# ChenJiahao031008/EAO-Fusion

Hardware: AMD Instinct MI355X
Metric: ORB kpts/s (640x480, 1k feat) + local-BA residuals/s (20 KF x 3k pts) (higher is better)
Workload: dtype u8; 1 GPU; ORBextractor FAST+rBRIEF, 640x480, 8-level pyramid, nFeatures 1000, batch=64 synthetic frames per GPU (BASELINE configs[1]); parallelism=frames sharded per GPU, no data-path collective

## Files before the change

eao_fusion_amd/csrc/orb.hip:

```cpp
#include "orb_internal.h"

using namespace eao::orb;

namespace {

__constant__ __align__(16) signed char c_pattern[1024] = {
#include "orb_pattern.inc"
};

constexpr int kResizeRows = 4;
__device__ __forceinline__ unsigned udot2w(unsigned a, unsigned b) {
    typedef unsigned short us2 __attribute__((ext_vector_type(2)));
    return __builtin_amdgcn_udot2(__builtin_bit_cast(us2, a), __builtin_bit_cast(us2, b), 0u, false);
}

struct ResizeLevel { int w, h, pitch, off; };
struct ResizeArgs {
    ResizeLevel D, S;
    double invX, invY;
    int srcIsInput;
    int pyrFrameBytes;
    int G;
    float invG;
    int frameAffinity;
// ... 465 lines not shown
                const int pos = total + __popcll(km & ((1ull << lane) - 1));
                if (pos < cellCap) out[pos] = (unsigned)(x + 3 + c.offX) | ((unsigned)(y + 3 + c.offY) << 12) | ((unsigned)v << 24);
            }
            total += __popcll(km);
        }
        if (total > 0 || pass == 1) {
            if (lane == 0) cellcnt[slot] = min(total, cellCap);
            return;
        }
    }
#undef QDIV
}

__device__ __forceinline__ int reflect101(int p, int len) {
    while (p < 0 || p >= len) p = p < 0 ? -p : 2 * len - 2 - p;
    return p;
}

typedef unsigned short u16x2 __attribute__((ext_vector_type(2)));
__device__ __forceinline__ unsigned udot2(unsigned a, unsigned b, unsigned c) {
    return __builtin_amdgcn_udot2(__builtin_bit_cast(u16x2, a), __builtin_bit_cast(u16x2, b), c, false);
}

struct BlurEdge {
    int off0;
    bool left;
    unsigned selA, selB, selC;
};

__device__ __forceinline__ BlurEdge blur_edge(int x4, int w) {
    BlurEdge e;
    const int wi = x4 >> 2, wmax = (w - 1) >> 2;
    const int wi0 = min(max(wi - 1, 0), wmax - 2);
    e.off0 = 4 * wi0;
    e.left = wi == 0;
    e.selA = e.selB = e.selC = 0;
#pragma unroll
    for (int k = 0; k < 12; k++) {
        int x = min(max(x4 - 4 + k, -3), w + 2);
        x = x < 0 ? -x : x;
        x = min(x, 2 * w - 2 - x);
        const int m = min(max(x - 4 * wi0, 0), 11);
        if (k < 4) e.selA |= (unsigned)min(m, 7) << (8 * k);
        else {
            const unsigned q = (unsigned)min(max(e.left ? m : m - 4, 0), 7) << (8 * (k & 3));
            if (k < 8) e.selB |= q; else e.selC |= q;
        }
    }
    return e;
}

template <int MODE>
__device__ __forceinline__ void blur_load(const uint8_t* __restrict__ base, unsigned rowOff, int x4, int w, const BlurEdge& e, unsigned L[3]) {
    const uint8_t* row = base + rowOff;
    if (MODE == 0) {
        const unsigned* q = reinterpret_cast<const unsigned*>(base + (rowOff + (unsigned)(x4 - 4)));
        L[0] = q[0]; L[1] = q[1]; L[2] = q[2];
    } else if (MODE == 1) {
        const unsigned* q = reinterpret_cast<const unsigned*>(base + (rowOff + (unsigned)e.off0));
        L[0] = q[0]; L[1] = q[1]; L[2] = q[2];
    } else {
        L[0] = L[1] = L[2] = 0;
#pragma unroll
        for (int k = 1; k < 11; k++) L[k >> 2] |= (unsigned)row[reflect101(x4 - 4 + k, w)] << (8 * (k & 3));
    }
}

template <int MODE>
__device__ __forceinline__ void blur_hpass(const unsigned L[3], const BlurEdge& e, unsigned hres[4]) {
    unsigned W0 = L[0], W1 = L[1], W2 = L[2];
    if (MODE == 1) {
        const unsigned a = e.left ? L[0] : L[1], b = e.left ? L[1] : L[2];
        W0 = __builtin_amdgcn_perm(L[1], L[0], e.selA);
        W1 = __builtin_amdgcn_perm(b, a, e.selB);
        W2 = __builtin_amdgcn_perm(b, a, e.selC);
    }
    constexpr unsigned T0 = 18u | 34u << 8 | 49u << 16 | 55u << 24, T1 = 49u | 34u << 8 | 18u << 16;
    hres[0] = __builtin_amdgcn_udot4(__builtin_amdgcn_alignbyte(W1, W0, 1), T0, __builtin_amdgcn_udot4(__builtin_amdgcn_alignbyte(W2, W1, 1), T1, 0, false), false);
    hres[1] = __builtin_amdgcn_udot4(__builtin_amdgcn_alignbyte(W1, W0, 2), T0, __builtin_amdgcn_udot4(__builtin_amdgcn_alignbyte(W2, W1, 2), T1, 0, false), false);
    hres[2] = __builtin_amdgcn_udot4(__builtin_amdgcn_alignbyte(W1, W0, 3), T0, __builtin_amdgcn_udot4(__builtin_amdgcn_alignbyte(W2, W1, 3), T1, 0, false), false);
    hres[3] = __builtin_amdgcn_udot4(W1, T0, __builtin_amdgcn_udot4(W2, T1, 0, false), false);
}

template <int MODE>
__device__ __forceinline__ void blur_strip(const uint8_t* __restrict__ src, int pitch, uint8_t* __restrict__ dst, int dpitch, int x4, int y0, int w, int h) {
    BlurEdge e = {};
    if (MODE == 1) e = blur_edge(x4, w);
    constexpr int NP = (kBlurRows + 6) / 2;
    constexpr int PF = MODE == 2 ? 1 : 3;
    unsigned raw[NP][2][3];
    auto fetch = [&](int m) {
#pragma unroll
        for (int q = 0; q < 2; q++) {
            int t = y0 - 3 + 2 * m + q;
            t = t < 0 ? -t : t;
            t = min(t, 2 * h - 2 - t);
            blur_load<MODE>(src, __umul24(t, pitch), x4, w, e, raw[m][q]);
        }
    };
#pragma unroll
    for (int m = 0; m < PF; m++) fetch(m);
    unsigned P[4][4];
#pragma unroll
    for (int m = 0; m < NP; m++) {
        if (m + PF < NP) fetch(m + PF);
        unsigned hr[2][4];
        blur_hpass<MODE>(raw[m][0], e, hr[0]);
        blur_hpass<MODE>(raw[m][1], e, hr[1]);
#pragma unroll
        for (int i = 0; i < 4; i++) P[m & 3][i] = hr[0][i] | (hr[1][i] << 16);
        if (m >= 3) {
#pragma unroll
            for (int q = 0; q < 2; q++) {
                const unsigned K0 = q ? 18u << 16 : (18u | 34u << 16), K1 = q ? (34u | 49u << 16) : (49u | 55u << 16),
                               K2 = q ? (55u | 49u << 16) : (49u | 34u << 16), K3 = q ? (34u | 18u << 16) : 18u;
                unsigned sv[4];
#pragma unroll
                for (int i = 0; i < 4; i++)
                    sv[i] = udot2(P[(m - 3) & 3][i], K0, udot2(P[(m - 2) & 3][i], K1, udot2(P[(m - 1) & 3][i], K2, udot2(P[m & 3][i], K3, 32768u))));
                const u16x2 lim = {255, 255};
                const u16x2 pa = __builtin_elementwise_min(__builtin_bit_cast(u16x2, __builtin_amdgcn_perm(sv[1], sv[0], 0x07060302u)), lim);
                const u16x2 pb = __builtin_elementwise_min(__builtin_bit_cast(u16x2, __builtin_amdgcn_perm(sv[3], sv[2], 0x07060302u)), lim);
                const unsigned packed = __builtin_amdgcn_perm(__builtin_bit_cast(unsigned, pb), __builtin_bit_cast(unsigned, pa), 0x06040200u);
                const int y = y0 + 2 * (m - 3) + q;
                *reinterpret_cast<unsigned*>(dst + (unsigned)(__umul24(y, dpitch) + x4)) = packed;
            }
        }
    }
}

__global__ __launch_bounds__(256) void k_blur7(const Geom* __restrict__ g, ImgSrc s, uint8_t* __restrict__ blur, int f0, int src0Aligned, int frameAffinity) {
    const int lane = threadIdx.x & 31;
    int f = blockIdx.y, bxi = blockIdx.x;
    if (frameAffinity) {
        const unsigned b = blockIdx.x + gridDim.x * blockIdx.y, xcd = b & 7, slot = b >> 3;
        f = (int)(xcd + 8 * (slot / gridDim.x)); bxi = (int)(slot % gridDim.x);
    }
    f += f0;
    int l = 0;
    while (l + 1 < g->nlevels && bxi >= g->L[l + 1].tileBase) l++;
    const LevelGeom L = g->L[l];
    const int strip = (bxi - L.tileBase) * kBlurStripsPerWg + (int)(threadIdx.x >> 5);
    const int x4 = (strip % L.tilesX) * kBlurSegW + lane * 4;
    const int y0 = (strip / L.tilesX) * kBlurRows;
    if (x4 >= L.w || y0 >= L.h) return;
    int pitch;
    const uint8_t* src = level_ptr(g, s, l, f, &pitch);
    uint8_t* dst = blur + (long long)f * g->pyrFrameBytes + L.off;
    if (l == 0 && !src0Aligned) blur_strip<2>(src, pitch, dst, L.pitch, x4, y0, L.w, L.h);
    else if (__any(x4 < 4 || x4 + 7 > L.w)) blur_strip<1>(src, pitch, dst, L.pitch, x4, y0, L.w, L.h);
    else blur_strip<0>(src, pitch, dst, L.pitch, x4, y0, L.w, L.h);
}

__device__ __forceinline__ int wave_sum_i32(int v) {
    v += __builtin_amdgcn_update_dpp(0, v, 0xB1, 0xF, 0xF, true);
    v += __builtin_amdgcn_update_dpp(0, v, 0x4E, 0xF, 0xF, true);
    v += __builtin_amdgcn_update_dpp(0, v, 0x141, 0xF, 0xF, true);
    v += __builtin_amdgcn_update_dpp(0, v, 0x140, 0xF, 0xF, true);
    v += __builtin_amdgcn_update_dpp(0, v, 0x142, 0xA, 0xF, true);
    v += __builtin_amdgcn_update_dpp(0, v, 0x143, 0xC, 0xF, true);
    return __builtin_amdgcn_readlane(v, 63);
}

constexpr int kUmaxTab[17] = {15, 15, 15, 15, 14, 14, 14, 13, 13, 12, 11, 10, 9, 8, 6, 3, -1};

__device__ __forceinline__ void sincos_f32_via_f64(float angle, float* sn, float* cs) {
    const double x = (double)angle;
    const int k = (int)(x * 0.63661977236758134308 + 0.5);
    const double kd = (double)k;
    const double r = (x - kd * 1.57079632673412561417e+00) - kd * 6.07710050650619224932e-11;
    const double z = r * r;
    const double ps = -1.66666666666666324348e-01 + z * (8.33333333332248946124e-03 + z * (-1.98412698298579493134e-04 +
                      z * (2.75573137070700676789e-06 + z * (-2.50507602534068634195e-08 + z * 1.58969099521155010221e-10))));
    const double sr = r + r * z * ps;
    const double pc = 4.16666666666666019037e-02 + z * (-1.38888888888741095749e-03 + z * (2.48015872894767294178e-05 +
                      z * (-2.75573143513906633035e-07 + z * (2.08757232129817482790e-09 + z * -1.13596475577881948265e-11))));
    const double cr = 1.0 - 0.5 * z + z * z * pc;
    double sv, cv;
    switch (k & 3) {
        case 0: sv = sr; cv = cr; break;
        case 1: sv = cr; cv = -sr; break;
        case 2: sv = -sr; cv = -cr; break;
        default: sv = -cr; cv = sr; break;
    }
    *sn = (float)sv;
    *cs = (float)cv;
}

__device__ __forceinline__ float fast_atan2_deg(float y, float x) {
    const float p1 = 0.9997878412794807f * (float)(180 / 3.1415926535897932384626433832795);
    const float p3 = -0.3258083974640975f * (float)(180 / 3.1415926535897932384626433832795);
    const float p5 = 0.1555786518463281f * (float)(180 / 3.1415926535897932384626433832795);
    const float p7 = -0.04432655554792128f * (float)(180 / 3.1415926535897932384626433832795);
    const float eps = (float)2.2204460492503131e-16;
    const float ax = fabsf(x), ay = fabsf(y);
    float a, c, c2;
    if (ax >= ay) {
        c = ay / (ax + eps);
        c2 = c * c;
        a = (((p7 * c2 + p5) * c2 + p3) * c2 + p1) * c;
    } else {
        c = ax / (ay + eps);
        c2 = c * c;
        a = 90.f - (((p7 * c2 + p5) * c2 + p3) * c2 + p1) * c;
    }
    if (x < 0) a = 180.f - a;
    if (y < 0) a = 360.f - a;
    return a;
}

__global__ __launch_bounds__(256) void k_orient_describe(const Geom* __restrict__ g, ImgSrc s, const uint8_t* __restrict__ blur,
                                                         const unsigned* __restrict__ levelkps, const int* __restrict__ levelcnt,
                                                         eao_keypoint* __restrict__ kps, uint8_t* __restrict__ desc,
                                                         int* __restrict__ nout, int cap, int f0, int nlevels, int lFirst, int lEnd, int writeN) {
    const int lane = threadIdx.x & 63, wv = __builtin_amdgcn_readfirstlane(threadIdx.x >> 6);
    unsigned pat[4];
#pragma unroll
    for (int k = 0; k < 4; k++) pat[k] = reinterpret_cast<const unsigned*>(c_pattern)[lane + 64 * k];
    int bx = blockIdx.x, fy = blockIdx.y;
    if ((gridDim.y & 7) == 0) {
        const unsigned b = blockIdx.x + gridDim.x * blockIdx.y, xcd = b & 7, slot = b >> 3;
        fy = (int)(xcd + 8 * (slot / gridDim.x));
        bx = (int)(slot % gridDim.x);
    }
    int j = bx * 4 + wv;
    const int f = fy + f0;
    int total, l, lbase;
    {
        int inc = lane < lEnd ? levelcnt[f * nlevels + lane] : 0;
        inc += __builtin_amdgcn_update_dpp(0, inc, 0x111, 0xF, 0xF, true);
        inc += __builtin_amdgcn_update_dpp(0, inc, 0x112, 0xF, 0xF, true);
        inc += __builtin_amdgcn_update_dpp(0, inc, 0x114, 0xF, 0xF, true);
        inc += __builtin_amdgcn_update_dpp(0, inc, 0x118, 0xF, 0xF, true);
        total = __builtin_amdgcn_readlane(inc, 15);
        if (lFirst > 0) j += __builtin_amdgcn_readlane(inc, lFirst - 1);
        l = (int)__popcll(__ballot(lane < nlevels && inc <= j));
        lbase = l > 0 ? __builtin_amdgcn_readlane(inc, min(l, kMaxLevels) - 1) : 0;
    }
    const int jout = j;
    if (writeN && bx == 0 && threadIdx.x == 0) nout[f] = min(total, cap);
    if (l >= nlevels || jout >= cap) return;
    j -= lbase;
    const LevelGeom L = g->L[l];
    const unsigned key = levelkps[(long long)f * g->totalKpCap + L.kpBase + j];
    const int cx = (int)(key & 0xFFF) + kMinBorder, cy = (int)((key >> 12) & 0xFFF) + kMinBorder;
    int pitch;
    const uint8_t* img = level_ptr(g, s, l, f, &pitch);
    constexpr int kPR = 18, kPW = 10;
    __shared__ unsigned patch[4][(2 * kPR + 1) * kPW];
    const int ph = (cx - kPR) & 3;
    const uint8_t* bw = blur + (long long)f * g->pyrFrameBytes + L.off + (cy - kPR) * L.pitch + (cx - kPR - ph);
    unsigned pw[6];
#pragma unroll
    for (int k = 0; k < 6; k++) {
        const int i = min(lane + 64 * k, (2 * kPR + 1) * kPW - 1), r = (i * 6554) >> 16;
        pw[k] = *reinterpret_cast<const unsigned*>(bw + (unsigned)(r * L.pitch + 4 * (i - r * kPW)));
    }
    constexpr int kMR = 15, kMW = 9;
    __shared__ unsigned mpatch[4][(2 * kMR + 1) * kMW];
    const bool imgAligned = ((((uintptr_t)img | (uintptr_t)pitch) & 3) == 0);
    const int mph = (cx - kMR) & 3;
    if (imgAligned) {
        const uint8_t* mw = img + (cy - kMR) * pitch + (cx - kMR - mph);
        unsigned mv[5];
#pragma unroll
        for (int k = 0; k < 5; k++) {
            const int i = min(lane + 64 * k, (2 * kMR + 1) * kMW - 1), r = (i * 7282) >> 16;
            mv[k] = *reinterpret_cast<const unsigned*>(mw + (unsigned)(r * pitch + 4 * (i - r * kMW)));
        }
#pragma unroll
        for (int k = 0; k < 5; k++)
            if (lane + 64 * k < (2 * kMR + 1) * kMW) mpatch[wv][lane + 64 * k] = mv[k];
    } else {
        uint8_t* mb = reinterpret_cast<uint8_t*>(mpatch[wv]);
        for (int i = lane; i < (2 * kMR + 1) * (2 * kMR + 1); i += 64) {
            const int r = i / (2 * kMR + 1), c = i - r * (2 * kMR + 1);
            mb[r * (4 * kMW) + c + mph] = img[(long long)(cy - kMR + r) * pitch + cx - kMR + c];
        }
    }
    eao::wave_sync();
    const int u = (lane & 31) - 15, half = lane >> 5;
    int m10 = 0, m01 = 0;
    if (u <= 15) {
        const uint8_t* c0 = reinterpret_cast<const uint8_t*>(mpatch[wv]) + kMR * (4 * kMW) + kMR + mph + u;
        const int au = u < 0 ? -u : u;
        auto row = [&](auto kc) {
            constexpr int k = decltype(kc)::value;
            constexpr int umLo = kUmaxTab[15 - k], umHi = kUmaxTab[k + 1];
            const int v = half ? k + 1 : k - 15;
            const int um = half ? umHi : umLo;
            const int pix = c0[v * (4 * kMW)];
            const int val = au <= um ? pix : 0;
            m10 += u * val;
            m01 += v * val;
        };
#define EAO_ROW(K) row(std::integral_constant<int, K>{});
        EAO_ROW(0) EAO_ROW(1) EAO_ROW(2) EAO_ROW(3) EAO_ROW(4) EAO_ROW(5) EAO_ROW(6) EAO_ROW(7)
        EAO_ROW(8) EAO_ROW(9) EAO_ROW(10) EAO_ROW(11) EAO_ROW(12) EAO_ROW(13) EAO_ROW(14) EAO_ROW(15)
#undef EAO_ROW
    }
    m10 = wave_sum_i32(m10);
    m01 = wave_sum_i32(m01);
    const float angle = fast_atan2_deg((float)m01, (float)m10);
    const float factorPI = (float)(3.1415926535897932384626433832795 / 180.f);
    float a, b;
    sincos_f32_via_f64(angle * factorPI, &b, &a);
#pragma unroll
    for (int k = 0; k < 6; k++)
        if (lane + 64 * k < (2 * kPR + 1) * kPW) patch[wv][lane + 64 * k] = pw[k];
    eao::wave_sync();
    const uint8_t* bc = reinterpret_cast<const uint8_t*>(patch[wv]) + kPR * (4 * kPW) + kPR + ph;
    unsigned long long words[4];
#pragma unroll
    for (int k = 0; k < 4; k++) {
        const float xa = (float)(signed char)(pat[k] & 0xFF), ya = (float)(signed char)((pat[k] >> 8) & 0xFF);
        const float xb = (float)(signed char)((pat[k] >> 16) & 0xFF), yb = (float)(signed char)(pat[k] >> 24);
        const int ra = __float2int_rn(xa * b + ya * a), ca = __float2int_rn(xa * a - ya * b);
        const int rb = __float2int_rn(xb * b + yb * a), cb = __float2int_rn(xb * a - yb * b);
        const int t0 = bc[ra * (4 * kPW) + ca], t1 = bc[rb * (4 * kPW) + cb];
        words[k] = __ballot(t0 < t1);
    }
    if (lane == 0) {
        unsigned long long* d = reinterpret_cast<unsigned long long*>(desc + ((long long)f * cap + jout) * 32);
        d[0] = words[0]; d[1] = words[1]; d[2] = words[2]; d[3] = words[3];
        eao_keypoint kp;
        const float fxp = (float)cx, fyp = (float)cy;
        kp.x = l ? fxp * L.scale : fxp;
        kp.y = l ? fyp * L.scale : fyp;
        kp.size = (float)L.scaledPatch;
        kp.angle = angle;
        kp.response = (float)(key >> 24);
        kp.octave = l;
        kp.class_id = -1;
        kps[(long long)f * cap + jout] = kp;
    }
}

__global__ void k_unpack_cand(const unsigned* __restrict__ keys, int n, float* __restrict__ xyr) {
    const int i = blockIdx.x * blockDim.x + threadIdx.x;
    if (i < n) {
        const unsigned k = keys[i];
        xyr[3 * i] = (float)(k & 0xFFF);
        xyr[3 * i + 1] = (float)((k >> 12) & 0xFFF);
        xyr[3 * i + 2] = (float)(k >> 24);
    }
}


}

struct StereoArgs {
    int nl, nr, frame;
    const eao_keypoint* kl; const eao_keypoint* kr;
    const uint4* dl; const uint4* dr;
    const float* scale; const float* invScale;
    float mb, mbf;
    float* uRight; float* depth; int* sad;
};
__device__ __forceinline__ int px_reflect(const uint8_t* img, int pitch, int w, int h, int x, int y) {
    x = x < 0 ? -x : (x >= w ? 2 * w - 2 - x : x);
    y = y < 0 ? -y : (y >= h ? 2 * h - 2 - y : y);
    return img[(long long)y * pitch + x];
}
__global__ __launch_bounds__(256) void k_stereo_match(const Geom* __restrict__ g, ImgSrc sl, ImgSrc sr, StereoArgs A) {
    const int lane = threadIdx.x & 63;
    const int iL = blockIdx.x * 4 + (threadIdx.x >> 6);
    if (iL >= A.nl) return;
    const eao_keypoint kpL = A.kl[iL];
    const int levelL = kpL.octave;
    const float vL = kpL.y, uL = kpL.x;
    const int row = (int)vL;
    const float minZ = A.mb, minD = -3, maxD = A.mbf / minZ;
    const float minU = uL - maxD, maxU = uL - minD;
    float outU = -1.0f, outD = -1.0f;
    int outS = -1;
    if (!(maxU < 0)) {
        const uint4 a0 = A.dl[2 * iL], a1 = A.dl[2 * iL + 1];
        unsigned best = 0xFFFFFFFFu;
        for (int iR = lane; iR < A.nr; iR += 64) {
            const eao_keypoint kr = A.kr[iR];
            const float r = 2.0f * A.scale[kr.octave];
            const int maxr = (int)ceilf(kr.y + r), minr = (int)floorf(kr.y - r);
            if (row < minr || row > maxr) continue;
            if (kr.octave < levelL - 1 || kr.octave > levelL + 1) continue;
            if (!(kr.x >= minU && kr.x <= maxU)) continue;
            const uint4 b0 = A.dr[2 * iR], b1 = A.dr[2 * iR + 1];
            const unsigned d = __popc(a0.x ^ b0.x) + __popc(a0.y ^ b0.y) + __popc(a0.z ^ b0.z) + __popc(a0.w ^ b0.w) +
                               __popc(a1.x ^ b1.x) + __popc(a1.y ^ b1.y) + __popc(a1.z ^ b1.z) + __popc(a1.w ^ b1.w);
            best = min(best, (d << 16) | (unsigned)iR);
        }
        for (int dlt = 32; dlt >= 1; dlt >>= 1) best = min(best, (unsigned)__shfl_xor((int)best, dlt));
        const int bestDist = (int)(best >> 16);
        if (best != 0xFFFFFFFFu && bestDist < refc::TH_HIGH) {
            const int bestIdxR = (int)(best & 0xFFFF);
            const float uR0 = A.kr[bestIdxR].x;
            const float sf = A.invScale[levelL];
            const int suL = (int)roundf(uL * sf), svL = (int)roundf(vL * sf), suR0 = (int)roundf(uR0 * sf);
            const int w = 5, Lw = 5;
            int pl, pr;
            const uint8_t* imgL = level_ptr(g, sl, levelL, A.frame, &pl);
            const uint8_t* imgR = level_ptr(g, sr, levelL, A.frame, &pr);
            const int lw = g->L[levelL].w, lh = g->L[levelL].h;
            const float iniu = (float)(suR0 + Lw - w), endu = (float)(suR0 + Lw + w + 1);
            if (!(iniu < 0 || endu >= (float)lw)) {
                const int cL = px_reflect(imgL, pl, lw, lh, suL, svL);
                int dL0 = 0, dL1 = 0, px0x = 0, px0y = 0, px1x = 0, px1y = 0;
                const bool has1 = lane + 64 < 121;
                px0y = lane / 11; px0x = lane - px0y * 11;
                dL0 = px_reflect(imgL, pl, lw, lh, suL - w + px0x, svL - w + px0y) - cL;
                if (has1) {
                    px1y = (lane + 64) / 11; px1x = lane + 64 - px1y * 11;
                    dL1 = px_reflect(imgL, pl, lw, lh, suL - w + px1x, svL - w + px1y) - cL;
                }
                int dists[11];
                int bestSad = 0x7FFFFFFF, bestinc = 0;
#pragma unroll
                for (int inc = -5; inc <= 5; inc++) {
                    const int cR = px_reflect(imgR, pr, lw, lh, suR0 + inc, svL);
                    int sacc = abs(dL0 - (px_reflect(imgR, pr, lw, lh, suR0 + inc - w + px0x, svL - w + px0y) - cR));
                    if (has1) sacc += abs(dL1 - (px_reflect(imgR, pr, lw, lh, suR0 + inc - w + px1x, svL - w + px1y) - cR));
                    for (int dlt = 32; dlt >= 1; dlt >>= 1) sacc += __shfl_xor(sacc, dlt);
                    dists[inc + 5] = sacc;
                    if (sacc < bestSad) { bestSad = sacc; bestinc = inc; }
                }
                if (!(bestinc == -Lw || bestinc == Lw)) {
                    float dist1 = 0, dist2 = 0, dist3 = 0;
#pragma unroll
                    for (int k = 0; k < 11; k++) {
                        if (k == Lw + bestinc - 1) dist1 = (float)dists[k];
                        if (k == Lw + bestinc) dist2 = (float)dists[k];
                        if (k == Lw + bestinc + 1) dist3 = (float)dists[k];
                    }
                    const float deltaR = (dist1 - dist3) / (2.0f * (dist1 + dist3 - 2.0f * dist2));
                    if (!(deltaR < -1 || deltaR > 1)) {
                        float bestuR = A.scale[levelL] * ((float)suR0 + (float)bestinc + deltaR);
                        float disparity = uL - bestuR;
                        if (disparity >= 0 && disparity < maxD) {
                            if (disparity <= 0) { disparity = 0.01f; bestuR = uL - 0.01f; }
                            outD = A.mbf / disparity;
                            outU = bestuR;
                            outS = bestSad;
                        }
                    }
                }
            }
        }
    }
    if (lane == 0) { A.uRight[iL] = outU; A.depth[iL] = outD; A.sad[iL] = outS; }
}

namespace eao {
namespace orb {

eao_status enqueue(eao_orb* h, const uint8_t* d_img, int pitch0, long long fs0, int batch, eao_keypoint* d_kps,
                   uint8_t* d_desc, int cap, int* d_n, hipStream_t st) {
    const Geom& g = h->geom;
    eao::Range rAll("eao_orb_extract: enqueue");
    ImgSrc s;
    s.img0 = d_img; s.pitch0 = pitch0; s.fs0 = fs0; s.pyr = h->d_pyr.p;
    h->lastSrc = s; h->lastBatch = batch; h->lastComplete = false; h->pyrFrame = -1;
    const bool prof = h->profiling;
    hipEvent_t* ev = nullptr;
    if (prof) {
        if (h->evUsed + kProfEvents > h->evs.size()) {
            const size_t old = h->evs.size();
            h->evs.resize(old + kProfEvents * 16, nullptr);
            for (size_t i = old; i < h->evs.size(); i++) EAO_HIP(hipEventCreate(&h->evs[i]));
        }
        ev = &h->evs[h->evUsed];
        h->evUsed += kProfEvents;
        EAO_HIP(hipEventRecord(ev[0], st));
    }
    eao_status so;
    if (h->evLastValid && h->lastStream != st) {
        if ((so = order_behind_last_call(h, st))) return so;
    }
    h->lastStream = st;
    EAO_HIP(hipEventRecord(h->evStart, st));
    const hipStream_t ss = h->side;
    const int cells0 = g.L[0].nCells;
    const bool early0 = !prof && g.nlevels > 1 && g.L[0].cellBase == 0 && cells0 < g.totalCells;
    const int aff = (batch & 7) == 0 ? 1 : 0;
    auto fast = [&](hipStream_t str, int first, int end) {
        eao::Range rg("orb: FAST cells");
        const bool whole = first == 0 && end == g.totalCells, narrow = g.fastStride == 48;
        auto* kern = whole ? (narrow ? k_fast_cells<true, 48> : k_fast_cells<true, kTileStrideWide>)
                           : (narrow ? k_fast_cells<false, 48> : k_fast_cells<false, kTileStrideWide>);
        hipLaunchKernelGGL(kern, dim3(128 * ((end - first + 127) / 128), batch), dim3(64), g.fastLdsBytes, str, h->d_geom.p, h->d_cells.p, s,
                           h->d_cellcand.p, h->d_cellcnt.p, 0, first, end, aff);
    };
    const int mid = early0 && batch >= 48 && g.nlevels > 3 ? 3 : 0;
    const bool qtEarly = mid > 0 && batch <= 96;
    const int src0Aligned = ((((uintptr_t)s.img0 | (uintptr_t)s.pitch0 | (uintptr_t)(batch > 1 ? s.fs0 : 0)) & 3) == 0) ? 1 : 0;
    auto quadtree = [&](hipStream_t str, int lFirst, int nLev) {
        eao::Range rg("orb: quad-tree");
        launch_quadtree(h, str, batch, 0, lFirst, nLev);
    };
    auto blur = [&]() -> eao_status {
        EAO_HIP(hipStreamWaitEvent(ss, h->evFork, 0));
        if (prof) EAO_HIP(hipEventRecord(ev[6], ss));
        { eao::Range rg("orb: blur"); hipLaunchKernelGGL(k_blur7, dim3(g.totalTiles, batch), dim3(256), 0, ss, h->d_geom.p, s, h->d_blur.p, 0, src0Aligned, aff); }
        if (prof) EAO_HIP(hipEventRecord(ev[7], ss));
        EAO_HIP(hipEventRecord(h->evJoin, ss));
        return EAO_OK;
    };
    if (h->pyrFused && batch <= 32) {
        auto pyramid = [&] {
            eao::Range rg("orb: pyramid");
            hipLaunchKernelGGL(k_pyramid_fused, dim3(h->pyr.tilesX * h->pyr.tilesY, 1, batch), dim3(kPyrThreads), h->pyrLds, st, h->pyr, s, 0);
        };
        if (prof) {
            pyramid();
            EAO_HIP(hipEventRecord(ev[1], st));
            EAO_HIP(hipEventRecord(h->evFork, st));
            if ((so = blur())) return so;
            EAO_HIP(hipStreamWaitEvent(st, h->evJoin, 0));
            EAO_HIP(hipEventRecord(ev[9], st));
            fast(st, 0, g.totalCells);
            EAO_HIP(hipEventRecord(ev[2], st));
            quadtree(st, 0, g.nlevels);
            EAO_HIP(hipEventRecord(ev[3], st));
            EAO_HIP(hipEventRecord(ev[4], st));
        } else {
            EAO_HIP(hipStreamWaitEvent(ss, h->evStart, 0));
            fast(ss, 0, cells0);
            quadtree(ss, 0, 1);
            pyramid();
            EAO_HIP(hipEventRecord(h->evFork, st));
            if ((so = blur())) return so;
            fast(st, cells0, g.totalCells);
            quadtree(st, 1, g.nlevels - 1);
            EAO_HIP(hipStreamWaitEvent(st, h->evJoin, 0));
        }
    } else {
        if (early0) {
            EAO_HIP(hipStreamWaitEvent(ss, h->evStart, 0));
            fast(ss, 0, cells0);
        }
        for (int l = 1; l < g.nlevels; l++) {
            const int G4 = eao::cdiv(g.L[l].w, 4);
            ResizeArgs ra;
            ra.G = G4; ra.invG = 1.0f / (float)G4;
            ra.D = {g.L[l].w, g.L[l].h, g.L[l].pitch, g.L[l].off};
            ra.S = {g.L[l - 1].w, g.L[l - 1].h, g.L[l - 1].pitch, g.L[l - 1].off};
            ra.invX = 1. / ((double)g.L[l].w / g.L[l - 1].w); ra.invY = 1. / ((double)g.L[l].h / g.L[l - 1].h);
            ra.srcIsInput = l == 1; ra.pyrFrameBytes = g.pyrFrameBytes;
            ra.frameAffinity = aff;
            { eao::Range rg("orb: pyramid"); hipLaunchKernelGGL(k_resize, dim3(eao::cdiv(G4 * eao::cdiv(g.L[l].h, kResizeRows), 64), 1, batch), dim3(64), 0, st, ra, s, 0); }
            if (l == mid - 1) {
                EAO_HIP(hipEventRecord(h->evMid, st));
                EAO_HIP(hipStreamWaitEvent(ss, h->evMid, 0));
                fast(ss, cells0, g.L[mid].cellBase);
                if (qtEarly) quadtree(ss, 0, mid);
            }
        }
        if (early0) EAO_HIP(hipEventRecord(h->evFast0, ss));
        if (prof) {
            EAO_HIP(hipEventRecord(ev[1], st));
            EAO_HIP(hipEventRecord(h->evFork, st));
            if ((so = blur())) return so;
            EAO_HIP(hipStreamWaitEvent(st, h->evJoin, 0));
            EAO_HIP(hipEventRecord(ev[9], st));
            fast(st, 0, g.totalCells);
            EAO_HIP(hipEventRecord(ev[2], st));
        } else {
            EAO_HIP(hipEventRecord(h->evFork, st));
            fast(st, early0 ? (mid ? g.L[mid].cellBase : cells0) : 0, g.totalCells);
            if ((so = blur())) return so;
            if (early0 && !qtEarly) EAO_HIP(hipStreamWaitEvent(st, h->evFast0, 0));
        }
        quadtree(st, qtEarly ? mid : 0, g.nlevels - (qtEarly ? mid : 0));
        if (prof) EAO_HIP(hipEventRecord(ev[3], st));
        EAO_HIP(hipStreamWaitEvent(st, h->evJoin, 0));
        if (prof) EAO_HIP(hipEventRecord(ev[4], st));
    }
    { eao::Range rg("orb: orientation + description"); hipLaunchKernelGGL(k_orient_describe, dim3(eao::cdiv(std::min(cap, g.totalKpCap), 4), batch), dim3(256), 0, st,
                       h->d_geom.p, s, h->d_blur.p, h->d_levelkps.p, h->d_levelcnt.p, d_kps, d_desc, d_n, cap, 0, g.nlevels, 0, g.nlevels, 1); }
    if (prof) {
        EAO_HIP(hipEventRecord(ev[5], st));
        EAO_HIP(hipEventRecord(ev[8], st));
    }
    h->evLastValid = true;
    if (h->everyCallEvent) { EAO_HIP(hipEventRecord(h->evLast, st)); h->evLastRecorded = true; }
    EAO_HIP(hipGetLastError());
    return EAO_OK;
}

__global__ __launch_bounds__(256) void k_stream_download(const uint4* __restrict__ src, uint4* __restrict__ dst, size_t n16) {
    for (size_t i = (size_t)blockIdx.x * 256 + threadIdx.x; i < n16; i += (size_t)gridDim.x * 256) dst[i] = src[i];
}

struct PyrExportLevel { int w, h, srcPitch, srcOff, dstPitch, rowChunks, chunkBase; long long dstOff; };
struct PyrExportArgs { int nlevels, border, totalChunks, pyrFrameBytes; PyrExportLevel L[kMaxLevels]; };
__global__ __launch_bounds__(256) void k_pyramid_export(PyrExportArgs A, ImgSrc s, int frame, uint8_t* __restrict__ dst) {
    const int idx = blockIdx.x * 256 + threadIdx.x;
    if (idx >= A.totalChunks) return;
    int l = 0;
    while (l + 1 < A.nlevels && idx >= A.L[l + 1].chunkBase) l++;
    const PyrExportLevel& L = A.L[l];
    const int r = idx - L.chunkBase, row = r / L.rowChunks, ch = r - row * L.rowChunks;
    const uint8_t* src = l == 0 ? s.img0 + (long long)frame * s.fs0 : s.pyr + (long long)frame * A.pyrFrameBytes + L.srcOff;
    const int pitch = l == 0 ? s.pitch0 : L.srcPitch;
    int y = row - A.border;
    y = y < 0 ? -y : (y >= L.h ? 2 * L.h - 2 - y : y);
    y = min(max(y, 0), L.h - 1);
    const uint8_t* srow = src + (long long)y * pitch;
    unsigned w4[4];
#pragma unroll
    for (int q = 0; q < 4; q++) {
        unsigned v = 0;
#pragma unroll
        for (int b = 0; b < 4; b++) {
            int x = ch * 16 + q * 4 + b - A.border;
            x = x < 0 ? -x : (x >= L.w ? 2 * L.w - 2 - x : x);
            x = min(max(x, 0), L.w - 1);
            v |= (unsigned)srow[x] << (8 * b);
        }
        w4[q] = v;
    }
    *reinterpret_cast<uint4*>(dst + L.dstOff + (long long)row * L.dstPitch + ch * 16) = make_uint4(w4[0], w4[1], w4[2], w4[3]);
}

eao_status enqueue_pyramid_export(eao_orb* h, int frame, int border) {
    const Geom& g = h->geom;
    for (int l = 0; l < g.nlevels; l++) EAO_REQUIRE(border < g.L[l].w && border < g.L[l].h, "level %d is smaller than the border", l);
    PyrExportArgs A;
    A.nlevels = g.nlevels; A.border = border; A.pyrFrameBytes = g.pyrFrameBytes;
    size_t off = 0;
    int chunks = 0;
    for (int l = 0; l < g.nlevels; l++) {
        PyrExportLevel& L = A.L[l];
        L.w = g.L[l].w; L.h = g.L[l].h; L.srcPitch = g.L[l].pitch; L.srcOff = g.L[l].off;
        L.dstPitch = (L.w + 2 * border + 63) & ~63;
        L.rowChunks = L.dstPitch / 16; L.chunkBase = chunks; L.dstOff = (long long)off;
        chunks += L.rowChunks * (L.h + 2 * border);
        off = (off + (size_t)L.dstPitch * (L.h + 2 * border) + 255) & ~(size_t)255;
    }
    A.totalChunks = chunks;
    if (h->pinPyrCap < off) {
        EAO_HIP(eao::wait_latency(h->stream));
        if (h->pinPyr) (void)hipHostFree(h->pinPyr);
        h->pinPyr = nullptr; h->pinPyrCap = 0;
        EAO_HIP(hipHostMalloc((void**)&h->pinPyr, off, hipHostMallocMapped));
        h->pinPyrCap = off;
    }
    unsigned char* dv = nullptr;
    EAO_HIP(hipHostGetDevicePointer((void**)&dv, h->pinPyr, 0));
    hipLaunchKernelGGL(k_pyramid_export, dim3(eao::cdiv(chunks, 256)), dim3(256), 0, h->stream, A, h->lastSrc, frame, dv);
    for (int l = 0; l < g.nlevels; l++) {
        h->pyrViews[l].data = h->pinPyr + A.L[l].dstOff + (size_t)border * A.L[l].dstPitch + border;
        h->pyrViews[l].width = A.L[l].w; h->pyrViews[l].height = A.L[l].h; h->pyrViews[l].step = A.L[l].dstPitch;
    }
    h->pyrFrame = frame; h->pyrBorder = border;
    return EAO_OK;
}

}
}

extern "C" {


eao_status eao_orb_stream_submit(eao_orb* h, int32_t slot, int32_t batch) {
    EAO_REQUIRE(h && slot >= 0 && slot < (int)h->slots.size(), "no such slot (eao_orb_stream_create first)");
    EAO_REQUIRE(batch >= 1 && batch <= h->sB, "a slot holds 1..%d frames", h->sB);
    eao_orb::StreamSlot& sl = h->slots[slot];
    if (sl.submitted) EAO_HIP(hipEventSynchronize(sl.evOut));
    eao_status st = ensure(h, h->sW, h->sH, h->sB);
    if (st) return st;
    const size_t B = batch;
    EAO_HIP(hipMemcpyAsync(sl.dIn, sl.pinIn, B * (size_t)h->sPitch * h->sH, hipMemcpyHostToDevice, h->sUp));
    EAO_HIP(hipEventRecord(sl.evIn, h->sUp));
    EAO_HIP(hipStreamWaitEvent(h->sRun, sl.evIn, 0));
    st = enqueue(h, sl.dIn, h->sPitch, (long long)h->sPitch * h->sH, batch, (eao_keypoint*)(sl.dOut + h->sOffK), sl.dOut + h->sOffD, h->sCap, (int*)sl.dOut, h->sRun);
    if (st) return st;
    EAO_HIP(hipEventRecord(sl.evDone, h->sRun));
    EAO_HIP(hipStreamWaitEvent(h->sDown, sl.evDone, 0));
    const size_t parts[3][2] = {{0, (B * sizeof(int) + 15) & ~(size_t)15}, {h->sOffK, B * (size_t)h->sCap * sizeof(eao_keypoint)}, {h->sOffD, B * (size_t)h->sCap * 32}};
    for (int q = 0; q < 3; q++) {
        const size_t n16 = (parts[q][1] + 15) / 16;
        const unsigned grid = (unsigned)std::min<size_t>((n16 + 255) / 256, 64);
        hipLaunchKernelGGL(k_stream_download, dim3(grid), dim3(256), 0, h->sDown, reinterpret_cast<const uint4*>(sl.dOut + parts[q][0]),
                           reinterpret_cast<uint4*>(sl.pinOutDev + parts[q][0]), n16);
    }
    EAO_HIP(hipEventRecord(sl.evOut, h->sDown));
    sl.batch = batch; sl.submitted = true;
    return EAO_OK;
}

eao_status eao_orb_level_candidates(eao_orb* h, int32_t frame, int32_t level, float* xyr, int32_t cap, int32_t* n) {
    EAO_REQUIRE(h && n && h->geomValid && h->lastBatch > 0, "no extraction has run on this handle");
    EAO_REQUIRE(frame >= 0 && frame < h->lastBatch && level >= 0 && level < h->geom.nlevels, "frame/level out of range");
    const Geom& g = h->geom;
    eao_status st0 = wait_last_extraction(h);
    if (st0) return st0;
    int cnt = 0;
    EAO_HIP(hipMemcpyAsync(&cnt, h->d_candcnt.p + frame * g.nlevels + level, sizeof(int), hipMemcpyDeviceToHost, h->stream));
    EAO_HIP(eao::wait_latency(h->stream));
    *n = cnt;
    if (!xyr || cnt == 0) return EAO_OK;
    const int m = std::min(cnt, cap);
    eao_status st = h->d_xyr.reserve((size_t)m * 3);
    if (st) return st;
    hipLaunchKernelGGL(k_unpack_cand, dim3(eao::cdiv(m, 256)), dim3(256), 0, h->stream,
                       h->d_cand.p + (long long)frame * g.totalCandCap + g.L[level].candBase, m, h->d_xyr.p);
    EAO_HIP(hipMemcpyAsync(xyr, h->d_xyr.p, (size_t)m * 3 * sizeof(float), hipMemcpyDeviceToHost, h->stream));
    EAO_HIP(eao::wait_latency(h->stream));
    return EAO_OK;
}


eao_status eao_compute_stereo_matches(eao_orb* left, eao_orb* right, int32_t frame, int32_t nl, const eao_keypoint* kps_l,
                                      const uint8_t* desc_l, int32_t nr, const eao_keypoint* kps_r, const uint8_t* desc_r,
                                      float mb, float mbf, float* u_right, float* depth) {
    EAO_REQUIRE(left && right && left->geomValid && right->geomValid && left->lastBatch > 0 && right->lastBatch > 0,
                "both extractors must have run on the stereo pair");
    EAO_REQUIRE(frame >= 0 && frame < left->lastBatch && frame < right->lastBatch, "frame out of range");
    const Geom& g = left->geom;
    EAO_REQUIRE(g.nlevels == right->geom.nlevels && g.L[0].w == right->geom.L[0].w && g.L[0].h == right->geom.L[0].h &&
                left->cfg.scale_factor == right->cfg.scale_factor, "the two extractors must share image size and pyramid");
    EAO_REQUIRE(nl >= 0 && nr >= 0 && nr < 65536 && (nl == 0 || (kps_l && desc_l && u_right && depth)) && (nr == 0 || (kps_r && desc_r)), "bad argument");
    for (int i = 0; i < nl; i++) {
        u_right[i] = -1.0f; depth[i] = -1.0f;
        EAO_REQUIRE(kps_l[i].octave >= 0 && kps_l[i].octave < g.nlevels, "left keypoint %d: octave out of range", i);
    }
    for (int i = 0; i < nr; i++) EAO_REQUIRE(kps_r[i].octave >= 0 && kps_r[i].octave < g.nlevels, "right keypoint %d: octave out of range", i);
    if (nl == 0 || nr == 0) return EAO_OK;
    eao_status stw = wait_last_extraction(left);
    if (!stw) stw = wait_last_extraction(right);
    if (stw) return stw;
// ... 48 lines not shown
```

Baseline: 253.3 million kpts/s.

## Process two keypoints per wave in ORB orientation/descriptor kernel

Restructures k_orient_describe so each 64-lane wave handles two keypoints, one per 32-lane half. Each half loads its patch windows with per-lane strided row loads, computes moments by folding symmetric rows (column sums for m10), and builds the 256-bit descriptor from eight 32-bit ballot halves. The grid is sized from per-level pair counts, and frame-to-XCD affinity becomes an explicit flag. This halves wave count and shared memory per keypoint, at the cost of more complex indexing and a pairing scheme that pads levels with odd counts.

Result: faster. 266.4 million kpts/s (median of 6 runs) (+5.2%).

```diff
diff --git a/eao_fusion_amd/csrc/orb.hip b/eao_fusion_amd/csrc/orb.hip
--- a/eao_fusion_amd/csrc/orb.hip
+++ b/eao_fusion_amd/csrc/orb.hip
@@ -641,17 +641,17 @@
     else blur_strip<0>(src, pitch, dst, L.pitch, x4, y0, L.w, L.h);
 }
 
-__device__ __forceinline__ int wave_sum_i32(int v) {
+__device__ __forceinline__ int half_sum_i32(int v, int half) {
     v += __builtin_amdgcn_update_dpp(0, v, 0xB1, 0xF, 0xF, true);
     v += __builtin_amdgcn_update_dpp(0, v, 0x4E, 0xF, 0xF, true);
     v += __builtin_amdgcn_update_dpp(0, v, 0x141, 0xF, 0xF, true);
     v += __builtin_amdgcn_update_dpp(0, v, 0x140, 0xF, 0xF, true);
     v += __builtin_amdgcn_update_dpp(0, v, 0x142, 0xA, 0xF, true);
-    v += __builtin_amdgcn_update_dpp(0, v, 0x143, 0xC, 0xF, true);
-    return __builtin_amdgcn_readlane(v, 63);
-}
-
-constexpr int kUmaxTab[17] = {15, 15, 15, 15, 14, 14, 14, 13, 13, 12, 11, 10, 9, 8, 6, 3, -1};
+    const int lo = __builtin_amdgcn_readlane(v, 31), hi = __builtin_amdgcn_readlane(v, 63);
+    return half ? hi : lo;
+}
+
+constexpr int kUmaxTab[16] = {15, 15, 15, 15, 14, 14, 14, 13, 13, 12, 11, 10, 9, 8, 6, 3};
 
 __device__ __forceinline__ void sincos_f32_via_f64(float angle, float* sn, float* cs) {
     const double x = (double)angle;
@@ -665,13 +665,9 @@
     const double pc = 4.16666666666666019037e-02 + z * (-1.38888888888741095749e-03 + z * (2.48015872894767294178e-05 +
                       z * (-2.75573143513906633035e-07 + z * (2.08757232129817482790e-09 + z * -1.13596475577881948265e-11))));
     const double cr = 1.0 - 0.5 * z + z * z * pc;
-    double sv, cv;
-    switch (k & 3) {
-        case 0: sv = sr; cv = cr; break;
-        case 1: sv = cr; cv = -sr; break;
-        case 2: sv = -sr; cv = -cr; break;
-        default: sv = -cr; cv = sr; break;
-    }
+    double sv = (k & 1) ? cr : sr, cv = (k & 1) ? sr : cr;
+    if (k & 2) sv = -sv;
+    if ((k + 1) & 2) cv = -cv;
     *sn = (float)sv;
     *cs = (float)cv;
 }
@@ -683,125 +679,138 @@
     const float p7 = -0.04432655554792128f * (float)(180 / 3.1415926535897932384626433832795);
     const float eps = (float)2.2204460492503131e-16;
     const float ax = fabsf(x), ay = fabsf(y);
-    float a, c, c2;
-    if (ax >= ay) {
-        c = ay / (ax + eps);
-        c2 = c * c;
-        a = (((p7 * c2 + p5) * c2 + p3) * c2 + p1) * c;
-    } else {
-        c = ax / (ay + eps);
-        c2 = c * c;
-        a = 90.f - (((p7 * c2 + p5) * c2 + p3) * c2 + p1) * c;
-    }
+    const bool ge = ax >= ay;
+    const float c = (ge ? ay : ax) / ((ge ? ax : ay) + eps);
+    const float c2 = c * c;
+    const float poly = (((p7 * c2 + p5) * c2 + p3) * c2 + p1) * c;
+    float a = ge ? poly : 90.f - poly;
     if (x < 0) a = 180.f - a;
     if (y < 0) a = 360.f - a;
     return a;
 }
 
+constexpr int kDescKp = 8;
+constexpr int kPR = 18, kPW = 10, kPRows = 2 * kPR + 1, kPLoads = (kPRows + 2) / 3;
+constexpr int kMR = 15, kMW = 9, kMRows = 2 * kMR + 1, kMLoads = (kMRows + 2) / 3;
+
 __global__ __launch_bounds__(256) void k_orient_describe(const Geom* __restrict__ g, ImgSrc s, const uint8_t* __restrict__ blur,
                                                          const unsigned* __restrict__ levelkps, const int* __restrict__ levelcnt,
                                                          eao_keypoint* __restrict__ kps, uint8_t* __restrict__ desc,
-                                                         int* __restrict__ nout, int cap, int f0, int nlevels, int lFirst, int lEnd, int writeN) {
+                                                         int* __restrict__ nout, int cap, int f0, int nlevels, int lFirst, int lEnd, int writeN,
+                                                         int frameAffinity) {
     const int lane = threadIdx.x & 63, wv = __builtin_amdgcn_readfirstlane(threadIdx.x >> 6);
-    unsigned pat[4];
-#pragma unroll
-    for (int k = 0; k < 4; k++) pat[k] = reinterpret_cast<const unsigned*>(c_pattern)[lane + 64 * k];
-    int bx = blockIdx.x, fy = blockIdx.y;
-    if ((gridDim.y & 7) == 0) {
-        const unsigned b = blockIdx.x + gridDim.x * blockIdx.y, xcd = b & 7, slot = b >> 3;
-        fy = (int)(xcd + 8 * (slot / gridDim.x));
-        bx = (int)(slot % gridDim.x);
-    }
-    int j = bx * 4 + wv;
+    const int hl = lane & 31, half = lane >> 5;
+    const int bx = frameAffinity ? (int)(blockIdx.x >> 3) : (int)blockIdx.x;
+    const int fy = frameAffinity ? (int)((blockIdx.x & 7) + 8 * blockIdx.y) : (int)blockIdx.y;
+    int p = bx * 4 + wv;
     const int f = fy + f0;
-    int total, l, lbase;
+    int total, l, kbase, pbase, cntl;
     {
-        int inc = lane < lEnd ? levelcnt[f * nlevels + lane] : 0;
-        inc += __builtin_amdgcn_update_dpp(0, inc, 0x111, 0xF, 0xF, true);
-        inc += __builtin_amdgcn_update_dpp(0, inc, 0x112, 0xF, 0xF, true);
-        inc += __builtin_amdgcn_update_dpp(0, inc, 0x114, 0xF, 0xF, true);
-        inc += __builtin_amdgcn_update_dpp(0, inc, 0x118, 0xF, 0xF, true);
-        total = __builtin_amdgcn_readlane(inc, 15);
-        if (lFirst > 0) j += __builtin_amdgcn_readlane(inc, lFirst - 1);
-        l = (int)__popcll(__ballot(lane < nlevels && inc <= j));
-        lbase = l > 0 ? __builtin_amdgcn_readlane(inc, min(l, kMaxLevels) - 1) : 0;
-    }
-    const int jout = j;
+        int cinc = lane < lEnd ? levelcnt[f * nlevels + lane] : 0;
+        int pinc = (cinc + 1) >> 1;
+        cinc += __builtin_amdgcn_update_dpp(0, cinc, 0x111, 0xF, 0xF, true);
+        pinc += __builtin_amdgcn_update_dpp(0, pinc, 0x111, 0xF, 0xF, true);
+        cinc += __builtin_amdgcn_update_dpp(0, cinc, 0x112, 0xF, 0xF, true);
+        pinc += __builtin_amdgcn_update_dpp(0, pinc, 0x112, 0xF, 0xF, true);
+        cinc += __builtin_amdgcn_update_dpp(0, cinc, 0x114, 0xF, 0xF, true);
+        pinc += __builtin_amdgcn_update_dpp(0, pinc, 0x114, 0xF, 0xF, true);
+        cinc += __builtin_amdgcn_update_dpp(0, cinc, 0x118, 0xF, 0xF, true);
+        pinc += __builtin_amdgcn_update_dpp(0, pinc, 0x118, 0xF, 0xF, true);
+        total = __builtin_amdgcn_readlane(cinc, 15);
+        if (lFirst > 0) p += __builtin_amdgcn_readlane(pinc, lFirst - 1);
+        l = (int)__popcll(__ballot(lane < nlevels && pinc <= p));
+        const int lprev = min(l, kMaxLevels) - 1;
+        pbase = l > 0 ? __builtin_amdgcn_readlane(pinc, lprev) : 0;
+        kbase = l > 0 ? __builtin_amdgcn_readlane(cinc, lprev) : 0;
+        cntl = __builtin_amdgcn_readlane(cinc, min(l, kMaxLevels - 1)) - kbase;
+    }
     if (writeN && bx == 0 && threadIdx.x == 0) nout[f] = min(total, cap);
-    if (l >= nlevels || jout >= cap) return;
-    j -= lbase;
+    const int j0 = 2 * (p - pbase);
+    if (l >= nlevels || kbase + j0 >= cap) return;
+    const bool hasB = j0 + 1 < cntl && kbase + j0 + 1 < cap;
     const LevelGeom L = g->L[l];
-    const unsigned key = levelkps[(long long)f * g->totalKpCap + L.kpBase + j];
+    const unsigned* lk = levelkps + (long long)f * g->totalKpCap + L.kpBase + j0;
+    const unsigned keyA = lk[0], keyB = lk[hasB ? 1 : 0];
+    const unsigned key = half ? keyB : keyA;
     const int cx = (int)(key & 0xFFF) + kMinBorder, cy = (int)((key >> 12) & 0xFFF) + kMinBorder;
     int pitch;
     const uint8_t* img = level_ptr(g, s, l, f, &pitch);
-    constexpr int kPR = 18, kPW = 10;
-    __shared__ unsigned patch[4][(2 * kPR + 1) * kPW];
+    __shared__ unsigned win[kDescKp][kPRows * kPW];
+    unsigned* wbuf = win[wv * 2 + half];
     const int ph = (cx - kPR) & 3;
-    const uint8_t* bw = blur + (long long)f * g->pyrFrameBytes + L.off + (cy - kPR) * L.pitch + (cx - kPR - ph);
-    unsigned pw[6];
-#pragma unroll
-    for (int k = 0; k < 6; k++) {
-        const int i = min(lane + 64 * k, (2 * kPR + 1) * kPW - 1), r = (i * 6554) >> 16;
-        pw[k] = *reinterpret_cast<const unsigned*>(bw + (unsigned)(r * L.pitch + 4 * (i - r * kPW)));
-    }
-    constexpr int kMR = 15, kMW = 9;
-    __shared__ unsigned mpatch[4][(2 * kMR + 1) * kMW];
+    const uint8_t* bw = blur + (long long)f * g->pyrFrameBytes + L.off;
+    unsigned pw[kPLoads];
+    {
+        const int pl = min(hl, 3 * kPW - 1);
+        const int r0 = pl >= 2 * kPW ? 2 : (pl >= kPW ? 1 : 0), w0 = pl - r0 * kPW;
+        const unsigned o0 = (unsigned)((cy - kPR + r0) * L.pitch + (cx - kPR - ph) + 4 * w0);
+        const unsigned step = (unsigned)(3 * L.pitch), olast = o0 + (unsigned)((kPRows - 1 - r0) * L.pitch);
+#pragma unroll
+        for (int k = 0; k < kPLoads; k++)
+            pw[k] = k < kPLoads - 1 ? *reinterpret_cast<const unsigned*>(bw + (unsigned)k * step + o0) : *reinterpret_cast<const unsigned*>(bw + olast);
+    }
     const bool imgAligned = ((((uintptr_t)img | (uintptr_t)pitch) & 3) == 0);
     const int mph = (cx - kMR) & 3;
     if (imgAligned) {
-        const uint8_t* mw = img + (cy - kMR) * pitch + (cx - kMR - mph);
-        unsigned mv[5];
-#pragma unroll
-        for (int k = 0; k < 5; k++) {
-            const int i = min(lane + 64 * k, (2 * kMR + 1) * kMW - 1), r = (i * 7282) >> 16;
-            mv[k] = *reinterpret_cast<const unsigned*>(mw + (unsigned)(r * pitch + 4 * (i - r * kMW)));
-        }
-#pragma unroll
-        for (int k = 0; k < 5; k++)
-            if (lane + 64 * k < (2 * kMR + 1) * kMW) mpatch[wv][lane + 64 * k] = mv[k];
+        const int ml = min(hl, 3 * kMW - 1);
+        const int r0 = ml >= 2 * kMW ? 2 : (ml >= kMW ? 1 : 0), w0 = ml - r0 * kMW;
+        const unsigned o0 = (unsigned)((cy - kMR + r0) * pitch + (cx - kMR - mph) + 4 * w0);
+        const unsigned step = (unsigned)(3 * pitch), olast = o0 + (unsigned)((kMRows - 1 - r0) * pitch);
+        unsigned mv[kMLoads];
+#pragma unroll
+        for (int k = 0; k < kMLoads; k++)
+            mv[k] = k < kMLoads - 1 ? *reinterpret_cast<const unsigned*>(img + (unsigned)k * step + o0) : *reinterpret_cast<const unsigned*>(img + olast);
+        if (hl < 3 * kMW) {
+#pragma unroll
+            for (int k = 0; k < kMLoads - 1; k++) wbuf[hl + 3 * kMW * k] = mv[k];
+            if (hl < kMW) wbuf[hl + 3 * kMW * (kMLoads - 1)] = mv[kMLoads - 1];
+        }
     } else {
-        uint8_t* mb = reinterpret_cast<uint8_t*>(mpatch[wv]);
-        for (int i = lane; i < (2 * kMR + 1) * (2 * kMR + 1); i += 64) {
-            const int r = i / (2 * kMR + 1), c = i - r * (2 * kMR + 1);
+        uint8_t* mb = reinterpret_cast<uint8_t*>(wbuf);
+#pragma clang loop vectorize(disable) interleave(disable) unroll(disable)
+        for (int i = hl; i < kMRows * kMRows; i += 32) {
+            const int r = i / kMRows, c = i - r * kMRows;
             mb[r * (4 * kMW) + c + mph] = img[(long long)(cy - kMR + r) * pitch + cx - kMR + c];
         }
     }
     eao::wave_sync();
-    const int u = (lane & 31) - 15, half = lane >> 5;
-    int m10 = 0, m01 = 0;
-    if (u <= 15) {
-        const uint8_t* c0 = reinterpret_cast<const uint8_t*>(mpatch[wv]) + kMR * (4 * kMW) + kMR + mph + u;
+    unsigned pat[8];
+#pragma unroll
+    for (int k = 0; k < 8; k++) pat[k] = reinterpret_cast<const unsigned*>(c_pattern)[hl + 32 * k];
+    const int u = hl - kMR;
+    int colsum = 0, m01 = 0;
+    if (hl < kMRows) {
+        const uint8_t* c0 = reinterpret_cast<const uint8_t*>(wbuf) + kMR * (4 * kMW) + kMR + mph + u;
         const int au = u < 0 ? -u : u;
-        auto row = [&](auto kc) {
-            constexpr int k = decltype(kc)::value;
-            constexpr int umLo = kUmaxTab[15 - k], umHi = kUmaxTab[k + 1];
-            const int v = half ? k + 1 : k - 15;
-            const int um = half ? umHi : umLo;
-            const int pix = c0[v * (4 * kMW)];
-            const int val = au <= um ? pix : 0;
-            m10 += u * val;
-            m01 += v * val;
+        colsum = c0[0];
+        auto rows = [&](auto vc) {
+            constexpr int v = decltype(vc)::value, um = kUmaxTab[v];
+            const int pp = c0[v * (4 * kMW)], pn = c0[-v * (4 * kMW)];
+            const bool in = um >= kMR || au <= um;
+            colsum += in ? pp + pn : 0;
+            m01 += v * (in ? pp - pn : 0);
         };
-#define EAO_ROW(K) row(std::integral_constant<int, K>{});
-        EAO_ROW(0) EAO_ROW(1) EAO_ROW(2) EAO_ROW(3) EAO_ROW(4) EAO_ROW(5) EAO_ROW(6) EAO_ROW(7)
-        EAO_ROW(8) EAO_ROW(9) EAO_ROW(10) EAO_ROW(11) EAO_ROW(12) EAO_ROW(13) EAO_ROW(14) EAO_ROW(15)
-#undef EAO_ROW
-    }
-    m10 = wave_sum_i32(m10);
-    m01 = wave_sum_i32(m01);
+#define EAO_ROWS(V) rows(std::integral_constant<int, V>{});
+        EAO_ROWS(1) EAO_ROWS(2) EAO_ROWS(3) EAO_ROWS(4) EAO_ROWS(5) EAO_ROWS(6) EAO_ROWS(7) EAO_ROWS(8)
+        EAO_ROWS(9) EAO_ROWS(10) EAO_ROWS(11) EAO_ROWS(12) EAO_ROWS(13) EAO_ROWS(14) EAO_ROWS(15)
+#undef EAO_ROWS
+    }
+    const int m10 = half_sum_i32(u * colsum, half);
+    m01 = half_sum_i32(m01, half);
     const float angle = fast_atan2_deg((float)m01, (float)m10);
     const float factorPI = (float)(3.1415926535897932384626433832795 / 180.f);
     float a, b;
     sincos_f32_via_f64(angle * factorPI, &b, &a);
-#pragma unroll
-    for (int k = 0; k < 6; k++)
-        if (lane + 64 * k < (2 * kPR + 1) * kPW) patch[wv][lane + 64 * k] = pw[k];
+    if (hl < 3 * kPW) {
+#pragma unroll
+        for (int k = 0; k < kPLoads - 1; k++) wbuf[hl + 3 * kPW * k] = pw[k];
+        if (hl < kPW) wbuf[hl + 3 * kPW * (kPLoads - 1)] = pw[kPLoads - 1];
+    }
     eao::wave_sync();
-    const uint8_t* bc = reinterpret_cast<const uint8_t*>(patch[wv]) + kPR * (4 * kPW) + kPR + ph;
-    unsigned long long words[4];
-#pragma unroll
-    for (int k = 0; k < 4; k++) {
+    const uint8_t* bc = reinterpret_cast<const uint8_t*>(wbuf) + kPR * (4 * kPW) + kPR + ph;
+    unsigned long long words[8];
+#pragma unroll
+    for (int k = 0; k < 8; k++) {
         const float xa = (float)(signed char)(pat[k] & 0xFF), ya = (float)(signed char)((pat[k] >> 8) & 0xFF);
         const float xb = (float)(signed char)((pat[k] >> 16) & 0xFF), yb = (float)(signed char)(pat[k] >> 24);
         const int ra = __float2int_rn(xa * b + ya * a), ca = __float2int_rn(xa * a - ya * b);
@@ -809,9 +818,14 @@
         const int t0 = bc[ra * (4 * kPW) + ca], t1 = bc[rb * (4 * kPW) + cb];
         words[k] = __ballot(t0 < t1);
     }
-    if (lane == 0) {
+    if (hl == 0 && (half == 0 || hasB)) {
+        const int jout = kbase + j0 + half;
+        unsigned w[8];
+#pragma unroll
+        for (int k = 0; k < 8; k++) w[k] = half ? (unsigned)(words[k] >> 32) : (unsigned)words[k];
         unsigned long long* d = reinterpret_cast<unsigned long long*>(desc + ((long long)f * cap + jout) * 32);
-        d[0] = words[0]; d[1] = words[1]; d[2] = words[2]; d[3] = words[3];
+#pragma unroll
+        for (int k = 0; k < 4; k++) d[k] = (unsigned long long)w[2 * k] | ((unsigned long long)w[2 * k + 1] << 32);
         eao_keypoint kp;
         const float fxp = (float)cx, fyp = (float)cy;
         kp.x = l ? fxp * L.scale : fxp;
@@ -993,6 +1007,14 @@
         EAO_HIP(hipEventRecord(h->evJoin, ss));
         return EAO_OK;
     };
+    auto describe = [&](hipStream_t str, int lFirst, int lEnd, int writeN) {
+        eao::Range rg("orb: orientation + description");
+        int pairs = 0;
+        for (int l = lFirst; l < lEnd; l++) pairs += eao::cdiv(g.L[l].listCap, 2);
+        const int gx = std::max(1, eao::cdiv(std::min(pairs, eao::cdiv(cap, 2) + g.nlevels), 4));
+        hipLaunchKernelGGL(k_orient_describe, aff ? dim3(8 * gx, batch / 8) : dim3(gx, batch), dim3(256), 0, str,
+                           h->d_geom.p, s, h->d_blur.p, h->d_levelkps.p, h->d_levelcnt.p, d_kps, d_desc, d_n, cap, 0, g.nlevels, lFirst, lEnd, writeN, aff);
+    };
     if (h->pyrFused && batch <= 32) {
         auto pyramid = [&] {
             eao::Range rg("orb: pyramid");
@@ -1063,8 +1085,7 @@
         EAO_HIP(hipStreamWaitEvent(st, h->evJoin, 0));
         if (prof) EAO_HIP(hipEventRecord(ev[4], st));
     }
-    { eao::Range rg("orb: orientation + description"); hipLaunchKernelGGL(k_orient_describe, dim3(eao::cdiv(std::min(cap, g.totalKpCap), 4), batch), dim3(256), 0, st,
-                       h->d_geom.p, s, h->d_blur.p, h->d_levelkps.p, h->d_levelcnt.p, d_kps, d_desc, d_n, cap, 0, g.nlevels, 0, g.nlevels, 1); }
+    describe(st, 0, g.nlevels, 1);
     if (prof) {
         EAO_HIP(hipEventRecord(ev[5], st));
         EAO_HIP(hipEventRecord(ev[8], st));
```
